# tiantianz/redpanda

Measured on AMD Instinct MI355X. Metric: validated+decoded batch GB/s per GPU and whole node; % of HBM peak, higher is better.
Workload: dtype u8

## Files before the change

redpanda_amd/csrc/rp_device.h:

```cpp
#pragma once

#include "rp_internal.h"

namespace rp {

#define DEV __device__ __forceinline__

DEV uint32_t lane() { return __lane_id(); }

DEV uint32_t wave_xor(uint32_t v) {
#pragma unroll
    for (int o = 32; o > 0; o >>= 1) v ^= __shfl_xor(v, o, 64);
    return v;
}
DEV uint32_t wave_or(uint32_t v) {
#pragma unroll
    for (int o = 32; o > 0; o >>= 1) v |= __shfl_xor(v, o, 64);
    return v;
}
DEV uint32_t rl(uint32_t v, int l) { return (uint32_t)__builtin_amdgcn_readlane((int)v, l); }
DEV uint32_t uni32(uint32_t v) { return (uint32_t)__builtin_amdgcn_readfirstlane((int)v); }
DEV uint64_t uni64(uint64_t v) {
    return (uint64_t)uni32((uint32_t)v) | ((uint64_t)uni32((uint32_t)(v >> 32)) << 32);
}
// ... 138 lines not shown
DEV uint32_t lbe32(const uint32_t (&w)[16], int k) { return __builtin_bswap32(l32(w, k)); }
DEV uint64_t lbe64(const uint32_t (&w)[16], int k) { return ((uint64_t)lbe32(w, k) << 32) | lbe32(w, k + 4); }
DEV uint32_t lbe16(const uint32_t (&w)[16], int k) { return (lb(w, k) << 8) | lb(w, k + 1); }

constexpr int wire_src(int l) {
    return (l >= 8 && l < 16) ? 15 - l
         : (l >= 17 && l < 21) ? 37 - l
         : (l >= 21 && l < 61) ? 21 + ((l < 23 ? 0 : l < 27 ? 2 : l < 35 ? 6 : l < 43 ? 14 : l < 51 ? 22 : l < 53 ? 30
                                        : l < 57 ? 32 : 36) +
                                       ((l < 23 ? 2 : l < 27 ? 4 : l < 35 ? 8 : l < 43 ? 8 : l < 51 ? 8 : l < 53 ? 2
                                        : 4) - 1 - (l - (l < 23 ? 21 : l < 27 ? 23 : l < 35 ? 27 : l < 43 ? 35
                                                         : l < 51 ? 43 : l < 53 ? 51 : l < 57 ? 53 : 57))))
         : 0;
}

DEV LHdr lane_header(uint32_t layout, const uint8_t* __restrict__ seg, uint64_t len, uint64_t p,
                     const uint32_t* __restrict__ th, uint32_t c57) {
    LHdr h;
    h.eof = 0;
    h.hcrc = h.computed = 0;
    h.size = 0;
    h.need = 0;
#pragma unroll
    for (int i = 0; i < 16; i++) h.w[i] = 0;
    const uint64_t rem = len - p;
    if (rem == 0) { h.status = RPGPU_ERRC_END_OF_STREAM; h.eof = 1; return h; }
    if (rem < RPGPU_HEADER_SIZE) { h.status = RPGPU_ERRC_INPUT_STREAM_NOT_ENOUGH_BYTES; h.eof = 1; return h; }
    lane_header_bytes(seg + p, h.w);
    uint32_t raw = 0;
    if (layout == RPGPU_LAYOUT_WIRE) {
        const uint32_t bl = lbe32(h.w, 8);
        if ((int64_t)(int32_t)bl + 12 < (int64_t)RPGPU_HEADER_SIZE) {
            h.status = RPGPU_ERRC_INPUT_STREAM_NOT_ENOUGH_BYTES;
            return h;
        }
        h.size = (int32_t)(bl + 12u);
        h.need = (uint32_t)((uint32_t)h.size - RPGPU_HEADER_SIZE);
#pragma unroll
        for (int k = 4; k < 61; k++) {
            const uint32_t d = (k < 8) ? (((uint32_t)h.size >> (8 * (k - 4))) & 0xFFu) : (k == 16) ? 1u : lb(h.w, wire_src(k));
            raw ^= th[(60 - k) * 256 + d];
        }
        h.computed = ~(c57 ^ raw);
        h.status = -1;
        return h;
    }
#pragma unroll
    for (int k = 4; k < 61; k++) raw ^= th[(60 - k) * 256 + lb(h.w, k)];
    h.computed = ~(c57 ^ raw);
    h.hcrc = h.w[0];
    h.size = (int32_t)h.w[1];
    h.need = (uint32_t)((uint32_t)h.size - RPGPU_HEADER_SIZE);
    if (h.hcrc == 0) { h.status = RPGPU_ERRC_FALLOCATED_FILE_READ_ZERO_BYTES_FOR_HEADER; return h; }
    if (h.hcrc != h.computed) { h.status = RPGPU_ERRC_HEADER_ONLY_CRC_MISSMATCH; return h; }
    h.status = -1;
    return h;
}

DEV uint32_t lane_prefix_raw(uint32_t layout, const uint32_t (&w)[16], const uint32_t* __restrict__ th) {
    uint32_t x = 0;
    if (layout == RPGPU_LAYOUT_WIRE) {
#pragma unroll
        for (int k = 21; k < 61; k++) x ^= th[(39 - (k - 21)) * 256 + lb(w, k)];
    } else {
#pragma unroll
        for (int k = 21; k < 61; k++) x ^= th[(39 - (wire_src(k) - 21)) * 256 + lb(w, k)];
    }
    return x;
}

// ... 134 lines not shown
```

redpanda_amd/csrc/rp_internal.h:

```cpp
#pragma once

#include <hip/hip_runtime.h>
#include <stdint.h>

#include "rpgpu.h"

namespace rp {

constexpr uint64_t kNone = ~0ull;
constexpr uint32_t kCrcPoly = 0x82F63B78u;

constexpr uint32_t kShiftLevels = 6;
constexpr uint32_t kBraidSkip = 1020;

constexpr uint32_t kVWaves = 16;
constexpr uint32_t kWinBytes = 16384;
constexpr uint32_t kLdsBraidOff = 0;
constexpr uint32_t kLdsSlice4Off = 131072;
constexpr uint32_t kLdsShiftOff = kLdsSlice4Off + 4096;
constexpr uint32_t kLdsValidateBytes = kLdsShiftOff + kShiftLevels * 4096;
static_assert(kLdsValidateBytes <= 160u * 1024u, "validate LDS image exceeds 160 KiB");

struct Tables {
    uint32_t slice[4][256];
// ... 119 lines not shown
constexpr size_t kCounterBytes = 256;

struct DeviceJob {
    const uint8_t* data;
    uint64_t data_len;
    const uint64_t* seg_off;
    const uint64_t* chunk_base;
    uint32_t n_segments;
    uint32_t flags;
    uint32_t layout;
    uint32_t chunk_bytes;
    uint32_t total_chunks;
    ChunkRec* chunks;
    uint64_t* chunk_count;
    uint64_t* chunk_entry;
    SegTerm* seg_term;
    rpgpu_batch_result* batches;
    uint64_t batch_capacity;
    uint64_t* slots;
    uint64_t* dcap;
    rpgpu_record_index* records;
    uint64_t record_capacity;
    uint8_t* decoded;
    uint64_t decoded_capacity;
    rpgpu_segment_summary* summaries;
    rpgpu_job_totals* totals;
    uint64_t* bitmap;
    const Tables* tables;
    uint32_t* counters;
    uint32_t* decode_list;
// ... 51 lines not shown
    uint64_t cap;
    uint32_t n;
    uint32_t ord;
    int32_t record_count;
    int32_t status;
};
hipError_t launch_host_desc(const DeviceJob& j, HostItem* items, uint32_t n, hipStream_t s);
hipError_t launch_host_gather(const DeviceJob& j, const HostItem* items, uint32_t n, uint8_t* stage, hipStream_t s);
hipError_t launch_host_patch(const DeviceJob& j, const HostItem* items, uint32_t n, hipStream_t s);
hipError_t launch_host_scatter(const DeviceJob& j, const HostItem* items, uint32_t n, const uint8_t* stage,
                               hipStream_t s);

hipError_t launch_chunk_base(const DeviceJob& j, hipStream_t s);
hipError_t launch_discover(const DeviceJob& j, hipStream_t s);
hipError_t launch_resolve(const DeviceJob& j, hipStream_t s);
hipError_t launch_emit(const DeviceJob& j, hipStream_t s);
hipError_t launch_validate(const DeviceJob& j, hipStream_t s, uint32_t grid, bool compose = true);
hipError_t launch_crc_compose(const DeviceJob& j, hipStream_t s, uint32_t grid);
bool dchain_wanted(const DeviceJob& j);
hipError_t launch_dchain(const DeviceJob& j, hipStream_t s, uint32_t grid);
hipError_t launch_validate_decoded(const DeviceJob& j, hipStream_t s, uint32_t grid);
hipError_t launch_walk(const DeviceJob& j, hipStream_t s, uint32_t grid);
hipError_t launch_decode(const DeviceJob& j, hipStream_t s, uint32_t grid);
hipError_t launch_decode_blocks(const DeviceJob& j, hipStream_t s, uint32_t grid);
hipError_t launch_lz_walk(const DeviceJob& j, hipStream_t s, uint32_t grid);
hipError_t launch_lz_exec(const DeviceJob& j, hipStream_t s);
hipError_t launch_raw_copy(const DeviceJob& j, hipStream_t s, uint32_t cus);
hipError_t launch_lzf_walk(const DeviceJob& j, hipStream_t s, uint32_t cus);
hipError_t launch_decode_finish(const DeviceJob& j, hipStream_t s, uint32_t grid, bool defer = false);
hipError_t launch_content_xxh(const DeviceJob& j, hipStream_t s, uint32_t grid);
hipError_t launch_content_apply(const DeviceJob& j, hipStream_t s, uint32_t grid);
// ... 79 lines not shown
```

redpanda_amd/csrc/rp_kernels.hip:

```cpp
#include "rp_device.h"

namespace rp {


#ifdef RPGPU_CHECKED
#include <cstdio>
#define RP_CHECK(flag, cond, fmt, ...)                                               \
    do {                                                                            \
        if (!(cond)) {                                                              \
            if (__lane_id() == 0) printf("RPGPU_CHECK %d " fmt "\n", __LINE__, __VA_ARGS__); \
            flag = true;                                                            \
        }                                                                           \
    } while (0)
#endif

DEV uint32_t find_segment(const uint64_t* __restrict__ chunk_base, uint32_t nseg, uint64_t g) {
    uint32_t lo = 0, hi = nseg;
    while (hi - lo > 1) {
        uint32_t mid = (lo + hi) >> 1;
        if (chunk_base[mid] <= g) lo = mid; else hi = mid;
    }
    return lo;
}

struct WalkOut {
    uint64_t exit;
    uint64_t tpos;
    uint32_t count;
    int32_t term;
};

DEV WalkOut wave_walk(uint32_t layout, const uint8_t* __restrict__ seg, uint64_t len, uint64_t p, uint64_t ce,
                      const Tables* __restrict__ T) {
    WalkOut w;
    w.count = 0;
    w.term = -1;
    w.tpos = 0;
    while (p < ce) {
        Hdr h = wave_header_of(layout, seg, len, p, T);
        if (h.status >= 0) { w.term = h.status | (h.eof << 8); w.tpos = p; break; }
        if (len - p - RPGPU_HEADER_SIZE < h.need) {
            w.count++;
            w.term = RPGPU_ERRC_INPUT_STREAM_NOT_ENOUGH_BYTES | (1 << 8);
            w.tpos = p;
            break;
        }
        w.count++;
        p += RPGPU_HEADER_SIZE + h.need;
    }
    w.exit = p;
    return w;
}

typedef uint32_t u32x4 __attribute__((ext_vector_type(4)));
struct ScanWin {
// ... 151 lines not shown
        exhausted = entry == kNone && se < ce;
    }
    if (lane() == 0) {
        ChunkRec r;
        r.entry = kNone;
        r.exit = kNone;
        r.count = 0;
        r.term = -1;
        r.tpos = 0;
        j.chunks[g] = r;
        j.chunk_entry[g] = entry != kNone ? entry : exhausted ? kExhausted : kNone;
    }
}

DEV WalkOut lane_walk(uint32_t layout, const uint8_t* __restrict__ seg, uint64_t len, uint64_t p, uint64_t ce,
                      const uint32_t* __restrict__ th, uint32_t c57) {
    WalkOut w;
    w.count = 0;
    w.term = -1;
    w.tpos = 0;
    while (p < ce) {
        const LHdr h = lane_header(layout, seg, len, p, th, c57);
        if (h.status >= 0) { w.term = h.status | (h.eof << 8); w.tpos = p; break; }
        if (len - p - RPGPU_HEADER_SIZE < h.need) {
            w.count++;
            w.term = RPGPU_ERRC_INPUT_STREAM_NOT_ENOUGH_BYTES | (1 << 8);
            w.tpos = p;
            break;
        }
        w.count++;
        p += RPGPU_HEADER_SIZE + h.need;
    }
    w.exit = p;
    return w;
}

__global__ __launch_bounds__(256) void k_chain(DeviceJob j) {
    extern __shared__ uint32_t th[];
// ... 5 lines not shown
    const uint32_t s = find_segment(j.chunk_base, j.n_segments, g);
    const uint64_t w = g - j.chunk_base[s];
    const uint64_t W = j.chunk_base[s + 1] - j.chunk_base[s];
    const uint64_t off = j.seg_off[s], len = j.seg_off[s + 1] - off;
    uint64_t p = entry;
    for (uint32_t k = 0;; k++) {
        const uint64_t cs = (w + k) * j.chunk_bytes;
        const uint64_t ce = (cs + j.chunk_bytes < len) ? cs + j.chunk_bytes : len;
        ChunkRec r;
        r.entry = kNone;
        r.exit = kNone;
        r.count = 0;
        r.term = -1;
        r.tpos = 0;
        if (p < ce) {
            const WalkOut o = lane_walk(j.layout, j.data + off, len, p, ce, th, j.tables->c57);
            r.entry = p;
            r.exit = o.exit;
            r.count = o.count;
            r.term = o.term;
            r.tpos = o.tpos;
            p = o.exit;
        }
        j.chunks[g + k] = r;
        if (r.term >= 0 || k + 1 >= kMaxCarry || w + k + 1 >= W || j.chunk_entry[g + k + 1] != kExhausted) break;
    }
}

__global__ __launch_bounds__(256) void k_resolve(DeviceJob j) {
    const uint32_t s = blockIdx.x;
    const uint32_t tid = threadIdx.x;
// ... 75 lines not shown
            continue;
        }
        const uint64_t wf = w0 + first;
        if (tid == first) s_pred = pred;
        __syncthreads();
        const uint64_t P = s_pred;
        if (tid < 64) {
            const uint64_t cs2 = wf * CS;
            const uint64_t ce2 = (cs2 + CS < len) ? cs2 + CS : len;
            WalkOut o;
            uint64_t entry = kNone;
            if (P >= ce2) {
                o.exit = P; o.count = 0; o.term = -1; o.tpos = 0;
            } else {
                entry = P;
                o = wave_walk(j.layout, seg, len, P, ce2, j.tables);
            }
            if (tid == 0) {
                ChunkRec nr;
                nr.entry = entry; nr.exit = o.exit; nr.count = o.count; nr.term = o.term; nr.tpos = o.tpos;
                j.chunks[c0 + wf] = nr;
                j.chunk_count[c0 + wf] = o.count;
                j.chunk_entry[c0 + wf] = entry;
                atomicAdd(&j.counters[0], 1u);
                if (o.term >= 0) {
                    s_st.pos = o.tpos; s_st.errc = o.term & 0xFF; s_st.eof = (o.term >> 8) & 1;
                    s_ended = 1;
                }
                s_T = o.exit;
            }
        }
        __syncthreads();
        w0 = wf + 1;
    }
    for (uint64_t w = w0 + tid; w < W; w += 256) {
        if (s_ended) {
            j.chunk_count[c0 + w] = 0;
            j.chunk_entry[c0 + w] = kNone;
        }
    }
    if (tid == 0) {
        if (!s_ended) { s_st.pos = s_T; s_st.errc = RPGPU_ERRC_END_OF_STREAM; s_st.eof = 1; }
        j.seg_term[s] = s_st;
    }
}

__global__ __launch_bounds__(256) void k_emit(DeviceJob j) {
    extern __shared__ uint32_t th[];
    init_lds_hdr(th, j.tables);
    const uint64_t g = (uint64_t)blockIdx.x * blockDim.x + threadIdx.x;
    if (g >= j.total_chunks) return;
    const uint64_t base_ord = j.chunk_count[g];
    const uint64_t cnt = j.chunk_count[g + 1] - base_ord;
    if (cnt == 0) return;
    const uint32_t s = find_segment(j.chunk_base, j.n_segments, g);
    const uint64_t off = j.seg_off[s], len = j.seg_off[s + 1] - off;
    const uint8_t* seg = j.data + off;
    const uint32_t c57 = j.tables->c57;
    const bool wire = j.layout == RPGPU_LAYOUT_WIRE;
    uint64_t p = j.chunk_entry[g];
    for (uint64_t i = 0; i < cnt; i++) {
#ifdef RPGPU_CHECKED
        if (!(p < len)) {
            printf("RPGPU_CHECK emit g=%llu i=%llu cnt=%llu p=%llu len=%llu\n", (unsigned long long)g,
                   (unsigned long long)i, (unsigned long long)cnt, (unsigned long long)p, (unsigned long long)len);
            break;
        }
#endif
        const LHdr h = lane_header(j.layout, seg, len, p, th, c57);
        const uint64_t ord = base_ord + i;
        const bool complete = (len - p - RPGPU_HEADER_SIZE) >= h.need;
        const uint32_t praw = lane_prefix_raw(j.layout, h.w, th);
        const uint32_t attrs = wire ? lbe16(h.w, 21) : l16(h.w, 21);
        const int32_t rc = (int32_t)(wire ? lbe32(h.w, 57) : l32(h.w, 57));
        const uint32_t codec = attrs & 7;
        uint64_t slots = 0, cap = 0;
        const bool decodable = (codec == RPGPU_CODEC_LZ4 || codec == RPGPU_CODEC_SNAPPY) && (j.flags & RPGPU_JOB_DECODE);
        if (complete) {
            if (codec == 0) {
                if ((j.flags & RPGPU_JOB_PARSE) && rc > 0 && (uint64_t)rc <= h.need) slots = (uint64_t)rc;
            } else if (decodable) {
                cap = decode_capacity_dev((int)codec, seg + p + RPGPU_HEADER_SIZE, h.need);
                if ((j.flags & RPGPU_JOB_PARSE) && rc > 0 && (uint64_t)rc <= cap) slots = (uint64_t)rc;
            }
        }
        if (ord < j.batch_capacity) {
            rpgpu_batch_result r;
            r.file_pos = p;
            uint32_t f = RPGPU_F_HEADER_OK;
            if (wire) {
                r.base_offset = (int64_t)lbe64(h.w, 0);
                r.first_timestamp = (int64_t)lbe64(h.w, 27);
                r.max_timestamp = (int64_t)lbe64(h.w, 35);
                r.producer_id = (int64_t)lbe64(h.w, 43);
                r.last_offset_delta = (int32_t)lbe32(h.w, 23);
                r.base_sequence = (int32_t)lbe32(h.w, 53);
                r.header_crc = 0;
                r.crc = lbe32(h.w, 17);
                r.producer_epoch = (int16_t)lbe16(h.w, 51);
                r.type = 1;
                if (lb(h.w, 16) == 2) f |= RPGPU_F_WIRE_V2;
            } else {
                r.base_offset = (int64_t)l64(h.w, 8);
                r.first_timestamp = (int64_t)l64(h.w, 27);
                r.max_timestamp = (int64_t)l64(h.w, 35);
                r.producer_id = (int64_t)l64(h.w, 43);
                r.last_offset_delta = (int32_t)l32(h.w, 23);
                r.base_sequence = (int32_t)l32(h.w, 53);
                r.header_crc = h.hcrc;
                r.crc = l32(h.w, 17);
                r.producer_epoch = (int16_t)l16(h.w, 51);
                r.type = (int8_t)lb(h.w, 16);
            }
            r.size_bytes = h.size;
            r.record_count = rc;
            r.crc_computed = 0;
            r.header_crc_computed = h.computed;
            if (complete) f |= RPGPU_F_COMPLETE;
            if (codec) f |= RPGPU_F_COMPRESSED;
            if (codec >= 5) f |= RPGPU_F_CODEC_INVALID;
            const bool host_codec = (j.flags & RPGPU_JOB_DECODE) && (j.flags & RPGPU_JOB_HOST_CODECS);
            if (complete && codec == RPGPU_CODEC_ZSTD && !(j.flags & RPGPU_JOB_DECODE)) f |= RPGPU_F_CODEC_UNSUPPORTED;
            r.flags = f;
            r.segment = s;
            r.index_base = off + p + RPGPU_HEADER_SIZE;
            r.decoded_off = 0;
            r.records_parsed = 0;
            r.decoded_len = (complete && codec == 0) ? (uint32_t)h.need : 0;
            r.decoded_crc = 0;
            r.decoded_header_crc = 0;
            r.attrs = (int16_t)attrs;
            r.parse_err = 0;
            r.reserved0 = 0;
            r.reserved1 = praw;
            j.batches[ord] = r;
            j.slots[ord] = slots;
            j.dcap[ord] = cap;
            if (complete && decodable) j.decode_list[atomicAdd(&j.counters[2], 1u)] = (uint32_t)ord;
            if (complete && (j.flags & RPGPU_JOB_DECODE) &&
                (codec == RPGPU_CODEC_GZIP || (codec == RPGPU_CODEC_ZSTD && !host_codec)))
                j.inf_list[atomicAdd(&j.counters[16], 1u)] = (uint32_t)ord;
            if (complete && codec == RPGPU_CODEC_ZSTD && host_codec)
                j.host_list[atomicAdd(&j.counters[19], 1u)] = (uint32_t)ord;
        }
        if (!complete) break;
        p += RPGPU_HEADER_SIZE + h.need;
    }
}

constexpr uint32_t kScanTile = 4096;

__global__ __launch_bounds__(256) void k_scan_tiles(uint64_t* data, const uint64_t* d_n, uint64_t n_host, uint64_t* tile_sums) {
    const uint64_t n = d_n ? (*d_n < n_host ? *d_n : n_host) : n_host;
    const uint64_t t0 = (uint64_t)blockIdx.x * kScanTile;
    if (t0 >= n) return;
    __shared__ uint64_t s[256];
    uint64_t v[16];
    uint64_t sum = 0;
    const uint64_t b = t0 + threadIdx.x * 16;
#pragma unroll
    for (int i = 0; i < 16; i++) {
// ... 5 lines not shown
    for (int o = 1; o < 256; o <<= 1) {
        uint64_t x = (threadIdx.x >= (uint32_t)o) ? s[threadIdx.x - o] : 0;
        __syncthreads();
        s[threadIdx.x] += x;
        __syncthreads();
    }
    uint64_t run = s[threadIdx.x] - sum;
#pragma unroll
    for (int i = 0; i < 16; i++) {
        if (b + i < n) data[b + i] = run;
        run += v[i];
    }
    if (threadIdx.x == 255) tile_sums[blockIdx.x] = s[255];
}

__global__ __launch_bounds__(1024) void k_scan_sums(uint64_t* tile_sums, const uint64_t* d_n, uint64_t n_host, uint64_t* total_out) {
    const uint64_t n = d_n ? (*d_n < n_host ? *d_n : n_host) : n_host;
    const uint64_t nt = (n + kScanTile - 1) / kScanTile;
    __shared__ uint64_t s[1024];
    __shared__ uint64_t carry;
    if (threadIdx.x == 0) carry = 0;
    __syncthreads();
    for (uint64_t t0 = 0; t0 < nt; t0 += 1024) {
        const uint64_t t = t0 + threadIdx.x;
        uint64_t v = t < nt ? tile_sums[t] : 0;
        s[threadIdx.x] = v;
        __syncthreads();
        for (int o = 1; o < 1024; o <<= 1) {
            uint64_t x = (threadIdx.x >= (uint32_t)o) ? s[threadIdx.x - o] : 0;
            __syncthreads();
            s[threadIdx.x] += x;
            __syncthreads();
        }
        if (t < nt) tile_sums[t] = carry + s[threadIdx.x] - v;
        __syncthreads();
        if (threadIdx.x == 1023) carry += s[1023];
        __syncthreads();
    }
    if (threadIdx.x == 0) total_out[0] = carry;
}

__global__ __launch_bounds__(256) void k_scan_add(uint64_t* data, const uint64_t* d_n, uint64_t n_host, const uint64_t* tile_sums) {
    const uint64_t n = d_n ? (*d_n < n_host ? *d_n : n_host) : n_host;
    const uint64_t t0 = (uint64_t)blockIdx.x * kScanTile;
    if (t0 >= n) return;
    const uint64_t add = tile_sums[blockIdx.x];
    for (uint64_t i = t0 + threadIdx.x; i < t0 + kScanTile && i < n; i += 256) data[i] += add;
}

__global__ __launch_bounds__(256) void k_finalize_segments(DeviceJob j) {
    const uint32_t s = blockIdx.x;
    const uint32_t tid = threadIdx.x;
    const uint64_t first = j.chunk_count[j.chunk_base[s]];
    const uint64_t last = j.chunk_count[j.chunk_base[s + 1]];
    const uint64_t cnt = last - first;
    const bool fits = last <= j.batch_capacity;
    const uint64_t fb = j.seg_first_bad[s];
    const uint64_t bad = (fits && fb < cnt) ? fb : cnt;
    const uint64_t upto = bad < cnt ? bad + (j.layout == RPGPU_LAYOUT_WIRE ? 0 : 1) : cnt;
    const uint64_t seg_len = j.seg_off[s + 1] - j.seg_off[s];
    __shared__ unsigned long long s_bytes, s_phys;
    if (tid == 0) { s_bytes = 0; s_phys = 0; }
    __syncthreads();
    if (fits) {
        if (seg_len < (1ull << 32)) {
            if (tid == 0) {
                if (upto > 0) {
// ... 52 lines not shown
        !(f & RPGPU_F_CODEC_OK))
        return false;
    if ((f & RPGPU_F_PARSED) && !(f & RPGPU_F_PARSE_OK)) return false;
    return true;
}

__global__ __launch_bounds__(256) void k_finalize_bitmap(DeviceJob j) {
    const uint64_t nb_total = j.chunk_count[j.total_chunks];
    const uint64_t nb = nb_total < j.batch_capacity ? nb_total : j.batch_capacity;
    const uint64_t b = (uint64_t)blockIdx.x * 256 + threadIdx.x;
    if ((b & ~63ull) >= nb) return;
    const uint64_t word = __ballot(b < nb && batch_valid(j.batches[b].flags, j.flags, j.layout));
    if ((threadIdx.x & 63) == 0) j.bitmap[b >> 6] = word;
}

__global__ void k_finalize_totals(DeviceJob j) {
    if (threadIdx.x != 0 || blockIdx.x != 0) return;
    const uint64_t nb_total = j.chunk_count[j.total_chunks];
    const uint64_t nb = nb_total < j.batch_capacity ? nb_total : j.batch_capacity;
    rpgpu_job_totals t;
    t.n_batches = nb_total;
    t.n_records = j.slots[nb];
    const uint64_t dtot = (j.flags & RPGPU_JOB_DECODE) ? j.dcap[nb] : 0;
    t.decoded_bytes = dtot;
    t.batch_capacity_needed = nb_total;
    t.record_capacity_needed = j.slots[nb];
    t.decoded_capacity_needed = dtot;
    uint32_t ov = j.counters[1];
    if (nb_total > j.batch_capacity) ov |= 1;
    if (j.slots[nb] > j.record_capacity) ov |= 2;
    if (dtot > j.decoded_capacity) ov |= 4;
    t.overflow = ov;
// ... 66 lines not shown
    return hipGetLastError();
}
hipError_t launch_host_patch(const DeviceJob& j, const HostItem* items, uint32_t n, hipStream_t s) {
    if (n) hipLaunchKernelGGL(k_host_patch, dim3((n + 255) / 256), dim3(256), 0, s, j, items, n);
    return hipGetLastError();
}
hipError_t launch_host_scatter(const DeviceJob& j, const HostItem* items, uint32_t n, const uint8_t* stage,
                               hipStream_t s) {
    if (n) hipLaunchKernelGGL(k_host_scatter, dim3((n + 3) / 4), dim3(256), 0, s, j, items, n, stage);
    return hipGetLastError();
}

__global__ __launch_bounds__(1024) void k_chunk_base(DeviceJob j) {
    __shared__ uint64_t sh[1024];
    __shared__ uint64_t carry;
    if (threadIdx.x == 0) carry = 0;
    __syncthreads();
    for (uint32_t b0 = 0; b0 < j.n_segments; b0 += 1024) {
        const uint32_t i = b0 + threadIdx.x;
        uint64_t v = 0;
        if (i < j.n_segments) {
            const uint64_t len = j.seg_off[i + 1] - j.seg_off[i];
            v = (len + j.chunk_bytes - 1) / j.chunk_bytes;
            if (v == 0) v = 1;
        }
        sh[threadIdx.x] = v;
        __syncthreads();
        for (int o = 1; o < 1024; o <<= 1) {
            uint64_t x = threadIdx.x >= (uint32_t)o ? sh[threadIdx.x - o] : 0;
            __syncthreads();
// ... 12 lines not shown
    hipLaunchKernelGGL(k_chunk_base, dim3(1), dim3(1024), 0, s, j);
    return hipGetLastError();
}

hipError_t launch_discover(const DeviceJob& j, hipStream_t s) {
    hipLaunchKernelGGL(k_discover, dim3((j.total_chunks + 3) / 4), dim3(256), 0, s, j);
    hipError_t e = hipGetLastError();
    if (e != hipSuccess) return e;
    hipLaunchKernelGGL(k_chain, dim3((j.total_chunks + 255) / 256), dim3(256), kLdsHdrBytes, s, j);
    return hipGetLastError();
}
hipError_t launch_resolve(const DeviceJob& j, hipStream_t s) {
    hipLaunchKernelGGL(k_resolve, dim3(j.n_segments), dim3(256), 0, s, j);
    return hipGetLastError();
}
hipError_t launch_emit(const DeviceJob& j, hipStream_t s) {
    hipLaunchKernelGGL(k_emit, dim3((j.total_chunks + 255) / 256), dim3(256), kLdsHdrBytes, s, j);
    return hipGetLastError();
}
hipError_t launch_finalize(const DeviceJob& j, hipStream_t s) {
    hipLaunchKernelGGL(k_finalize_segments, dim3(j.n_segments), dim3(256), 0, s, j);
    const uint64_t words = (j.batch_capacity + 63) / 64;
    if (j.bitmap) {
        const uint32_t grid = (uint32_t)((words * 64 + 255) / 256);
        hipLaunchKernelGGL(k_finalize_bitmap, dim3(grid ? grid : 1), dim3(256), 0, s, j);
    }
    hipLaunchKernelGGL(k_finalize_totals, dim3(1), dim3(64), 0, s, j);
    return hipGetLastError();
}

size_t scan_temp_bytes(uint64_t n) { return ((n + kScanTile - 1) / kScanTile + 1) * sizeof(uint64_t); }

hipError_t scan_exclusive_dev(uint64_t* data, const uint64_t* d_n, uint64_t n_cap, uint64_t* temp, hipStream_t s) {
    const uint32_t tiles = (uint32_t)((n_cap + kScanTile - 1) / kScanTile);
    const uint32_t g = tiles ? tiles : 1;
    hipLaunchKernelGGL(k_scan_tiles, dim3(g), dim3(256), 0, s, data, d_n, n_cap, temp);
    hipLaunchKernelGGL(k_scan_sums, dim3(1), dim3(1024), 0, s, temp, d_n, n_cap, temp + g);
    hipLaunchKernelGGL(k_scan_add, dim3(g), dim3(256), 0, s, data, d_n, n_cap, temp);
    return hipGetLastError();
}

__global__ void k_copy_total(uint64_t* data, const uint64_t* d_n, uint64_t n_host, const uint64_t* total) {
    const uint64_t n = d_n ? (*d_n < n_host ? *d_n : n_host) : n_host;
    data[n] = *total;
}

hipError_t scan_exclusive_u64(uint64_t* data, uint64_t n, void* temp, size_t temp_bytes, hipStream_t s) {
    (void)temp_bytes;
    uint64_t* t = (uint64_t*)temp;
    const uint32_t tiles = (uint32_t)((n + kScanTile - 1) / kScanTile);
    scan_exclusive_dev(data, nullptr, n, t, s);
    hipLaunchKernelGGL(k_copy_total, dim3(1), dim3(1), 0, s, data, (const uint64_t*)nullptr, n, t + (tiles ? tiles : 1));
    return hipGetLastError();
}

hipError_t scan_exclusive_u64_devn(uint64_t* data, const uint64_t* d_n, uint64_t n_cap, void* temp, hipStream_t s) {
    uint64_t* t = (uint64_t*)temp;
    const uint32_t tiles = (uint32_t)((n_cap + kScanTile - 1) / kScanTile);
    scan_exclusive_dev(data, d_n, n_cap, t, s);
    hipLaunchKernelGGL(k_copy_total, dim3(1), dim3(1), 0, s, data, d_n, n_cap, t + (tiles ? tiles : 1));
    return hipGetLastError();
}

}
```

redpanda_amd/csrc/rp_runtime.hip:

```cpp
#include <hip/hip_runtime.h>
#include <nmmintrin.h>

#include <algorithm>
#include <array>
#include <atomic>
#include <cstdio>
#include <cstdlib>
#include <cstring>
#include <mutex>
#include <random>
#include <string>
#include <thread>
#include <vector>

#include "rp_device.h"
#include "rp_hostcodec.h"

namespace rp {

static uint32_t raw_step_zero(uint32_t c, const uint32_t* t0) { return t0[c & 0xFF] ^ (c >> 8); }

static void build_tables(Tables* T) {
    uint32_t t0[256];
    for (uint32_t i = 0; i < 256; i++) {
// ... 575 lines not shown

int check_job(rpgpu_ctx* c, const rpgpu_job* job) {
    if (!c || !job || !job->d_data || !job->d_seg_offsets || !job->h_seg_offsets || job->n_segments == 0 ||
        !job->d_batches || !job->d_summaries || !job->d_totals)
        return fail(c, RPGPU_E_INVALID, "rpgpu_submit: missing argument");
    if (((uintptr_t)job->d_data & 15) != 0) return fail(c, RPGPU_E_INVALID, "rpgpu_submit: d_data must be 16-byte aligned");
    if (job->layout != RPGPU_LAYOUT_DISK && job->layout != RPGPU_LAYOUT_WIRE)
        return fail(c, RPGPU_E_INVALID, "rpgpu_submit: unknown layout");
    if ((job->flags & RPGPU_JOB_PARSE) && !job->d_records && job->record_capacity)
        return fail(c, RPGPU_E_INVALID, "rpgpu_submit: PARSE needs d_records");
    return RPGPU_OK;
}

struct Layout {
    uint64_t tc;
    uint64_t zcap, gcap, bl_cap, split_min, split_cap;
    size_t cbase, chunks, ccount, centry, segterm, slots, dcap, counters, dlist, slist, llist, fbad;
    size_t ilist, istate, ioff, itot, hlist, zitems, gzsmem, gzsit;
    size_t blocks, plans, pstate, longl, wlong, rawl, lanel, lzfl, lzft, split, spart, scan;
    size_t need;
};

Layout job_layout(const rpgpu_job* job, uint32_t cu_count) {
    Layout L;
    const uint32_t nseg = job->n_segments;
    const uint32_t cs = job->chunk_bytes ? job->chunk_bytes : (256u << 10);
    const uint64_t bcap = job->batch_capacity, data_len = job->h_seg_offsets[nseg];
    uint64_t tc = 0;
    for (uint32_t i = 0; i < nseg; i++) {
        const uint64_t len = job->h_seg_offsets[i + 1] - job->h_seg_offsets[i];
        uint64_t nc = (len + cs - 1) / cs;
        tc += nc ? nc : 1;
    }
    L.tc = tc;
    size_t off = 0;
    auto take = [&](size_t bytes) { size_t o = off; off = align_up(off + bytes, 256); return o; };
    L.cbase = take((nseg + 1) * 8);
    L.chunks = take(tc * sizeof(ChunkRec));
    L.ccount = take((tc + 1) * 8);
    L.centry = take(tc * 8);
    L.segterm = take(nseg * sizeof(SegTerm));
    L.slots = take((bcap + 1) * 8);
    L.dcap = take((bcap + 1) * 8);
    L.counters = take(kCounterBytes);
    L.dlist = take((bcap + 1) * 4);
    L.slist = take((bcap + 1) * 4);
    L.llist = take((bcap + 1) * 4);
    L.fbad = take((size_t)nseg * 4);
    const bool decode_job = (job->flags & RPGPU_JOB_DECODE) != 0;
    L.ilist = take(decode_job ? (bcap + 1) * 4 : 0);
    L.istate = take(decode_job ? (bcap + 1) * 4 : 0);
    L.ioff = take(decode_job ? (bcap + 1) * 8 : 0);
    L.itot = take(decode_job ? (bcap + 1) * 8 : 0);
    const bool host_job = decode_job && (job->flags & RPGPU_JOB_HOST_CODECS);
    L.hlist = take(host_job ? (bcap + 1) * 4 : 0);
// ... 38 lines not shown
    if (int rc = grow(c, c->ws, L.need, s, "workspace")) return rc;
    uint8_t* ws = c->ws.as<uint8_t>();

    j.data = job->d_data;
    j.data_len = data_len;
    j.seg_off = job->d_seg_offsets;
    j.chunk_base = (const uint64_t*)(ws + L.cbase);
    j.n_segments = nseg;
    j.flags = job->flags;
    j.layout = job->layout;
    j.chunk_bytes = job->chunk_bytes ? job->chunk_bytes : (256u << 10);
    j.total_chunks = (uint32_t)L.tc;
    j.chunks = (ChunkRec*)(ws + L.chunks);
    j.chunk_count = (uint64_t*)(ws + L.ccount);
    j.chunk_entry = (uint64_t*)(ws + L.centry);
    j.seg_term = (SegTerm*)(ws + L.segterm);
    j.batches = job->d_batches;
    j.batch_capacity = job->batch_capacity;
    j.slots = (uint64_t*)(ws + L.slots);
    j.dcap = (uint64_t*)(ws + L.dcap);
    j.records = job->d_records;
    j.record_capacity = job->d_records ? job->record_capacity : 0;
    j.decoded = job->d_decoded;
    j.decoded_capacity = job->d_decoded ? job->decoded_capacity : 0;
    j.summaries = job->d_summaries;
    j.totals = job->d_totals;
    j.bitmap = job->d_valid_bitmap;
    j.tables = c->d_tables;
    j.counters = (uint32_t*)(ws + L.counters);
    j.decode_list = (uint32_t*)(ws + L.dlist);
// ... 81 lines not shown
        HIPCHK(c, (call));                                                                 \
        if (diag().debug_sync) {                                                           \
            fprintf(stderr, "[rpgpu] stage %s\n", name);                                   \
            fflush(stderr);                                                                \
            hipError_t _e = hipStreamSynchronize(s);                                       \
            if (_e == hipSuccess && c->side.stream) _e = hipStreamSynchronize(c->side.stream);   \
            if (_e == hipSuccess && c->side2.stream) _e = hipStreamSynchronize(c->side2.stream); \
            if (_e != hipSuccess) return fail(c, RPGPU_E_HIP, "stage " name " failed", _e); \
        }                                                                                  \
    } while (0)

hipError_t mark(hipEvent_t* ev, int i, hipStream_t s) { return ev ? hipEventRecord(ev[i], s) : hipSuccess; }

int stage_discover(rpgpu_ctx* c, const DeviceJob& j, hipStream_t s, hipEvent_t* ev, uint64_t* scan_tmp, bool emit) {
    STAGE("chunk_base", launch_chunk_base(j, s));
    HIPCHK(c, hipMemsetAsync(j.counters, 0, kCounterBytes, s));
    HIPCHK(c, hipMemsetAsync(j.seg_first_bad, 0xFF, (size_t)j.n_segments * 4, s));
    STAGE("discover", launch_discover(j, s));
    HIPCHK(c, mark(ev, 1, s));
    STAGE("resolve", launch_resolve(j, s));
    STAGE("scan_chunks", scan_exclusive_u64(j.chunk_count, j.total_chunks, scan_tmp, 0, s));
    if (emit) STAGE("emit", launch_emit(j, s));
    return RPGPU_OK;
}

int stage_members(rpgpu_ctx* c, DeviceJob& j, hipStream_t s, uint64_t* scan_tmp) {
    const uint32_t cus = c->cu_count;
    if (j.flags & RPGPU_JOB_DECODE) {
        const bool split = j.inf_scratch && j.zs_fast;
        STAGE("zstamps", launch_zstamps(s, 0));
        Fork zfork;
        if (split) {
            j.zs_split = 1;
            HIPCHK(c, zfork.open(s, c->side));
            STAGE("zplan", launch_zplan(j, c->side.stream, cus * 4));
            STAGE("zparse", launch_zparse(j, c->side.stream, cus * 4));
            HIPCHK(c, zfork.end());
// ... 834 lines not shown
```

Before: 3600.

## Parallelize batch emit across recorded header positions and fold small launches

During the discover walk, the first K batch-header positions of each chunk are now recorded into a new chunk_pos array. The emit kernel then uses these to spread work across (chunk, index) items in a grid-stride loop with software-prefetched header loads, where previously one thread serially walked each whole chunk. It also removes two memsets by zeroing counters in k_chunk_base, drops the k_copy_total and k_finalize_totals launches by folding them into existing kernels, and stages segment tables in LDS. The cost is extra workspace and stores during the walk, and the K-th item must still walk any remaining batches serially.

```diff
diff --git a/redpanda_amd/csrc/rp_device.h b/redpanda_amd/csrc/rp_device.h
--- a/redpanda_amd/csrc/rp_device.h
+++ b/redpanda_amd/csrc/rp_device.h
@@ -176,6 +176,40 @@
          : 0;
 }
 
+DEV void lane_header_verdict(uint32_t layout, LHdr& h, const uint32_t* __restrict__ th, uint32_t c57) {
+    h.eof = 0;
+    h.hcrc = h.computed = 0;
+    h.size = 0;
+    h.need = 0;
+    uint32_t raw = 0;
+    if (layout == RPGPU_LAYOUT_WIRE) {
+        const uint32_t bl = lbe32(h.w, 8);
+        if ((int64_t)(int32_t)bl + 12 < (int64_t)RPGPU_HEADER_SIZE) {
+            h.status = RPGPU_ERRC_INPUT_STREAM_NOT_ENOUGH_BYTES;
+            return;
+        }
+        h.size = (int32_t)(bl + 12u);
+        h.need = (uint32_t)((uint32_t)h.size - RPGPU_HEADER_SIZE);
+#pragma unroll
+        for (int k = 4; k < 61; k++) {
+            const uint32_t d = (k < 8) ? (((uint32_t)h.size >> (8 * (k - 4))) & 0xFFu) : (k == 16) ? 1u : lb(h.w, wire_src(k));
+            raw ^= th[(60 - k) * 256 + d];
+        }
+        h.computed = ~(c57 ^ raw);
+        h.status = -1;
+        return;
+    }
+#pragma unroll
+    for (int k = 4; k < 61; k++) raw ^= th[(60 - k) * 256 + lb(h.w, k)];
+    h.computed = ~(c57 ^ raw);
+    h.hcrc = h.w[0];
+    h.size = (int32_t)h.w[1];
+    h.need = (uint32_t)((uint32_t)h.size - RPGPU_HEADER_SIZE);
+    if (h.hcrc == 0) { h.status = RPGPU_ERRC_FALLOCATED_FILE_READ_ZERO_BYTES_FOR_HEADER; return; }
+    if (h.hcrc != h.computed) { h.status = RPGPU_ERRC_HEADER_ONLY_CRC_MISSMATCH; return; }
+    h.status = -1;
+}
+
 DEV LHdr lane_header(uint32_t layout, const uint8_t* __restrict__ seg, uint64_t len, uint64_t p,
                      const uint32_t* __restrict__ th, uint32_t c57) {
     LHdr h;
@@ -189,33 +223,7 @@
     if (rem == 0) { h.status = RPGPU_ERRC_END_OF_STREAM; h.eof = 1; return h; }
     if (rem < RPGPU_HEADER_SIZE) { h.status = RPGPU_ERRC_INPUT_STREAM_NOT_ENOUGH_BYTES; h.eof = 1; return h; }
     lane_header_bytes(seg + p, h.w);
-    uint32_t raw = 0;
-    if (layout == RPGPU_LAYOUT_WIRE) {
-        const uint32_t bl = lbe32(h.w, 8);
-        if ((int64_t)(int32_t)bl + 12 < (int64_t)RPGPU_HEADER_SIZE) {
-            h.status = RPGPU_ERRC_INPUT_STREAM_NOT_ENOUGH_BYTES;
-            return h;
-        }
-        h.size = (int32_t)(bl + 12u);
-        h.need = (uint32_t)((uint32_t)h.size - RPGPU_HEADER_SIZE);
-#pragma unroll
-        for (int k = 4; k < 61; k++) {
-            const uint32_t d = (k < 8) ? (((uint32_t)h.size >> (8 * (k - 4))) & 0xFFu) : (k == 16) ? 1u : lb(h.w, wire_src(k));
-            raw ^= th[(60 - k) * 256 + d];
-        }
-        h.computed = ~(c57 ^ raw);
-        h.status = -1;
-        return h;
-    }
-#pragma unroll
-    for (int k = 4; k < 61; k++) raw ^= th[(60 - k) * 256 + lb(h.w, k)];
-    h.computed = ~(c57 ^ raw);
-    h.hcrc = h.w[0];
-    h.size = (int32_t)h.w[1];
-    h.need = (uint32_t)((uint32_t)h.size - RPGPU_HEADER_SIZE);
-    if (h.hcrc == 0) { h.status = RPGPU_ERRC_FALLOCATED_FILE_READ_ZERO_BYTES_FOR_HEADER; return h; }
-    if (h.hcrc != h.computed) { h.status = RPGPU_ERRC_HEADER_ONLY_CRC_MISSMATCH; return h; }
-    h.status = -1;
+    lane_header_verdict(layout, h, th, c57);
     return h;
 }
 
diff --git a/redpanda_amd/csrc/rp_internal.h b/redpanda_amd/csrc/rp_internal.h
--- a/redpanda_amd/csrc/rp_internal.h
+++ b/redpanda_amd/csrc/rp_internal.h
@@ -157,6 +157,8 @@
     ChunkRec* chunks;
     uint64_t* chunk_count;
     uint64_t* chunk_entry;
+    uint32_t* chunk_pos;
+    uint32_t chunk_pos_k;
     SegTerm* seg_term;
     rpgpu_batch_result* batches;
     uint64_t batch_capacity;
@@ -238,7 +240,7 @@
 hipError_t launch_chunk_base(const DeviceJob& j, hipStream_t s);
 hipError_t launch_discover(const DeviceJob& j, hipStream_t s);
 hipError_t launch_resolve(const DeviceJob& j, hipStream_t s);
-hipError_t launch_emit(const DeviceJob& j, hipStream_t s);
+hipError_t launch_emit(const DeviceJob& j, hipStream_t s, uint32_t cus);
 hipError_t launch_validate(const DeviceJob& j, hipStream_t s, uint32_t grid, bool compose = true);
 hipError_t launch_crc_compose(const DeviceJob& j, hipStream_t s, uint32_t grid);
 bool dchain_wanted(const DeviceJob& j);
diff --git a/redpanda_amd/csrc/rp_kernels.hip b/redpanda_amd/csrc/rp_kernels.hip
--- a/redpanda_amd/csrc/rp_kernels.hip
+++ b/redpanda_amd/csrc/rp_kernels.hip
@@ -31,7 +31,7 @@
 };
 
 DEV WalkOut wave_walk(uint32_t layout, const uint8_t* __restrict__ seg, uint64_t len, uint64_t p, uint64_t ce,
-                      const Tables* __restrict__ T) {
+                      const Tables* __restrict__ T, uint32_t* __restrict__ pos, uint64_t ps, uint32_t K, uint64_t cs) {
     WalkOut w;
     w.count = 0;
     w.term = -1;
@@ -39,6 +39,7 @@
     while (p < ce) {
         Hdr h = wave_header_of(layout, seg, len, p, T);
         if (h.status >= 0) { w.term = h.status | (h.eof << 8); w.tpos = p; break; }
+        if (w.count < K && lane() == 0) pos[w.count * ps] = (uint32_t)(p - cs);
         if (len - p - RPGPU_HEADER_SIZE < h.need) {
             w.count++;
             w.term = RPGPU_ERRC_INPUT_STREAM_NOT_ENOUGH_BYTES | (1 << 8);
@@ -220,7 +221,8 @@
 }
 
 DEV WalkOut lane_walk(uint32_t layout, const uint8_t* __restrict__ seg, uint64_t len, uint64_t p, uint64_t ce,
-                      const uint32_t* __restrict__ th, uint32_t c57) {
+                      const uint32_t* __restrict__ th, uint32_t c57, uint32_t* __restrict__ pos, uint64_t ps,
+                      uint32_t K, uint64_t cs) {
     WalkOut w;
     w.count = 0;
     w.term = -1;
@@ -228,6 +230,7 @@
     while (p < ce) {
         const LHdr h = lane_header(layout, seg, len, p, th, c57);
         if (h.status >= 0) { w.term = h.status | (h.eof << 8); w.tpos = p; break; }
+        if (w.count < K) pos[w.count * ps] = (uint32_t)(p - cs);
         if (len - p - RPGPU_HEADER_SIZE < h.need) {
             w.count++;
             w.term = RPGPU_ERRC_INPUT_STREAM_NOT_ENOUGH_BYTES | (1 << 8);
@@ -263,7 +266,8 @@
         r.term = -1;
         r.tpos = 0;
         if (p < ce) {
-            const WalkOut o = lane_walk(j.layout, j.data + off, len, p, ce, th, j.tables->c57);
+            const WalkOut o = lane_walk(j.layout, j.data + off, len, p, ce, th, j.tables->c57,
+                                        j.chunk_pos + (g + k), j.total_chunks, j.chunk_pos_k, cs);
             r.entry = p;
             r.exit = o.exit;
             r.count = o.count;
@@ -369,7 +373,8 @@
                 o.exit = P; o.count = 0; o.term = -1; o.tpos = 0;
             } else {
                 entry = P;
-                o = wave_walk(j.layout, seg, len, P, ce2, j.tables);
+                o = wave_walk(j.layout, seg, len, P, ce2, j.tables, j.chunk_pos + (c0 + wf), j.total_chunks,
+                              j.chunk_pos_k, cs2);
             }
             if (tid == 0) {
                 ChunkRec nr;
@@ -400,106 +405,190 @@
     }
 }
 
+DEV bool emit_batch(const DeviceJob& j, const uint32_t* __restrict__ th, const LHdr& h, uint32_t s, uint64_t off,
+                    uint64_t len, uint64_t p, uint64_t ord) {
+    const uint8_t* seg = j.data + off;
+    const bool wire = j.layout == RPGPU_LAYOUT_WIRE;
+    const bool complete = (len - p - RPGPU_HEADER_SIZE) >= h.need;
+    const uint32_t praw = lane_prefix_raw(j.layout, h.w, th);
+    const uint32_t attrs = wire ? lbe16(h.w, 21) : l16(h.w, 21);
+    const int32_t rc = (int32_t)(wire ? lbe32(h.w, 57) : l32(h.w, 57));
+    const uint32_t codec = attrs & 7;
+    uint64_t slots = 0, cap = 0;
+    const bool decodable = (codec == RPGPU_CODEC_LZ4 || codec == RPGPU_CODEC_SNAPPY) && (j.flags & RPGPU_JOB_DECODE);
+    if (complete) {
+        if (codec == 0) {
+            if ((j.flags & RPGPU_JOB_PARSE) && rc > 0 && (uint64_t)rc <= h.need) slots = (uint64_t)rc;
+        } else if (decodable) {
+            cap = decode_capacity_dev((int)codec, seg + p + RPGPU_HEADER_SIZE, h.need);
+            if ((j.flags & RPGPU_JOB_PARSE) && rc > 0 && (uint64_t)rc <= cap) slots = (uint64_t)rc;
+        }
+    }
+    if (ord < j.batch_capacity) {
+        rpgpu_batch_result r;
+        r.file_pos = p;
+        uint32_t f = RPGPU_F_HEADER_OK;
+        if (wire) {
+            r.base_offset = (int64_t)lbe64(h.w, 0);
+            r.first_timestamp = (int64_t)lbe64(h.w, 27);
+            r.max_timestamp = (int64_t)lbe64(h.w, 35);
+            r.producer_id = (int64_t)lbe64(h.w, 43);
+            r.last_offset_delta = (int32_t)lbe32(h.w, 23);
+            r.base_sequence = (int32_t)lbe32(h.w, 53);
+            r.header_crc = 0;
+            r.crc = lbe32(h.w, 17);
+            r.producer_epoch = (int16_t)lbe16(h.w, 51);
+            r.type = 1;
+            if (lb(h.w, 16) == 2) f |= RPGPU_F_WIRE_V2;
+        } else {
+            r.base_offset = (int64_t)l64(h.w, 8);
+            r.first_timestamp = (int64_t)l64(h.w, 27);
+            r.max_timestamp = (int64_t)l64(h.w, 35);
+            r.producer_id = (int64_t)l64(h.w, 43);
+            r.last_offset_delta = (int32_t)l32(h.w, 23);
+            r.base_sequence = (int32_t)l32(h.w, 53);
+            r.header_crc = h.hcrc;
+            r.crc = l32(h.w, 17);
+            r.producer_epoch = (int16_t)l16(h.w, 51);
+            r.type = (int8_t)lb(h.w, 16);
+        }
+        r.size_bytes = h.size;
+        r.record_count = rc;
+        r.crc_computed = 0;
+        r.header_crc_computed = h.computed;
+        if (complete) f |= RPGPU_F_COMPLETE;
+        if (codec) f |= RPGPU_F_COMPRESSED;
+        if (codec >= 5) f |= RPGPU_F_CODEC_INVALID;
+        const bool host_codec = (j.flags & RPGPU_JOB_DECODE) && (j.flags & RPGPU_JOB_HOST_CODECS);
+        if (complete && codec == RPGPU_CODEC_ZSTD && !(j.flags & RPGPU_JOB_DECODE)) f |= RPGPU_F_CODEC_UNSUPPORTED;
+        r.flags = f;
+        r.segment = s;
+        r.index_base = off + p + RPGPU_HEADER_SIZE;
+        r.decoded_off = 0;
+        r.records_parsed = 0;
+        r.decoded_len = (complete && codec == 0) ? (uint32_t)h.need : 0;
+        r.decoded_crc = 0;
+        r.decoded_header_crc = 0;
+        r.attrs = (int16_t)attrs;
+        r.parse_err = 0;
+        r.reserved0 = 0;
+        r.reserved1 = praw;
+        j.batches[ord] = r;
+        j.slots[ord] = slots;
+        j.dcap[ord] = cap;
+        if (complete && decodable) j.decode_list[atomicAdd(&j.counters[2], 1u)] = (uint32_t)ord;
+        if (complete && (j.flags & RPGPU_JOB_DECODE) &&
+            (codec == RPGPU_CODEC_GZIP || (codec == RPGPU_CODEC_ZSTD && !host_codec)))
+            j.inf_list[atomicAdd(&j.counters[16], 1u)] = (uint32_t)ord;
+        if (complete && codec == RPGPU_CODEC_ZSTD && host_codec)
+            j.host_list[atomicAdd(&j.counters[19], 1u)] = (uint32_t)ord;
+    }
+    return complete;
+}
+
+constexpr uint32_t kEmitSegs = 512;
+constexpr uint32_t kEmitWgsPerCu = 2;
+
+struct EmitRaw {
+    uint64_t c0, c1;
+    uint32_t pos;
+};
+struct EmitItem {
+    uint64_t ord, p, off, len, cnt;
+    uint32_t s, i;
+    bool live;
+};
+
 __global__ __launch_bounds__(256) void k_emit(DeviceJob j) {
     extern __shared__ uint32_t th[];
+    __shared__ uint64_t s_cb[kEmitSegs + 1], s_so[kEmitSegs + 1];
+    const bool staged = j.n_segments <= kEmitSegs;
+    if (staged)
+        for (uint32_t k = threadIdx.x; k <= j.n_segments; k += 256) { s_cb[k] = j.chunk_base[k]; s_so[k] = j.seg_off[k]; }
     init_lds_hdr(th, j.tables);
-    const uint64_t g = (uint64_t)blockIdx.x * blockDim.x + threadIdx.x;
-    if (g >= j.total_chunks) return;
-    const uint64_t base_ord = j.chunk_count[g];
-    const uint64_t cnt = j.chunk_count[g + 1] - base_ord;
-    if (cnt == 0) return;
-    const uint32_t s = find_segment(j.chunk_base, j.n_segments, g);
-    const uint64_t off = j.seg_off[s], len = j.seg_off[s + 1] - off;
-    const uint8_t* seg = j.data + off;
+    const uint64_t* cb = staged ? s_cb : j.chunk_base;
+    const uint64_t* so = staged ? s_so : j.seg_off;
     const uint32_t c57 = j.tables->c57;
-    const bool wire = j.layout == RPGPU_LAYOUT_WIRE;
-    uint64_t p = j.chunk_entry[g];
-    for (uint64_t i = 0; i < cnt; i++) {
+    const uint32_t K = j.chunk_pos_k;
+    const uint64_t n_items = (uint64_t)j.total_chunks * K;
+    const uint64_t stride = (uint64_t)gridDim.x * 256;
+    const uint64_t tc = j.total_chunks;
+
+    auto load_raw = [&](uint64_t it) {
+        EmitRaw r;
+        r.c0 = r.c1 = 0;
+        r.pos = 0;
+        if (it < n_items) {
+            const uint64_t g = it % tc;
+            r.c0 = j.chunk_count[g];
+            r.c1 = j.chunk_count[g + 1];
+            r.pos = j.chunk_pos[it];
+        }
+        return r;
+    };
+    auto resolve = [&](uint64_t it, const EmitRaw& r) {
+        const uint32_t i = (uint32_t)(it / tc);
+        const uint64_t g = it % tc;
+        EmitItem m;
+        m.cnt = r.c1 - r.c0;
+        m.live = i < m.cnt;
+        m.ord = r.c0 + i;
+        m.i = i;
+        m.s = 0;
+        m.p = m.off = m.len = 0;
+        if (m.live) {
+            m.s = find_segment(cb, j.n_segments, g);
+            m.off = so[m.s];
+            m.len = so[m.s + 1] - m.off;
+            m.p = (g - cb[m.s]) * j.chunk_bytes + r.pos;
+        }
+        return m;
+    };
+
+    uint64_t it = (uint64_t)blockIdx.x * 256 + threadIdx.x;
+    EmitItem cur = resolve(it, load_raw(it));
+    LHdr h;
+#pragma unroll
+    for (int k = 0; k < 16; k++) h.w[k] = 0;
+    if (cur.live) lane_header_bytes(j.data + cur.off + cur.p, h.w);
+    EmitRaw rn = load_raw(it + stride);
+    while (it < n_items) {
+        const EmitItem nxt = resolve(it + stride, rn);
+        uint32_t wn[16];
+#pragma unroll
+        for (int k = 0; k < 16; k++) wn[k] = 0;
+        if (nxt.live) lane_header_bytes(j.data + nxt.off + nxt.p, wn);
+        rn = load_raw(it + 2 * stride);
+        if (cur.live) {
 #ifdef RPGPU_CHECKED
-        if (!(p < len)) {
-            printf("RPGPU_CHECK emit g=%llu i=%llu cnt=%llu p=%llu len=%llu\n", (unsigned long long)g,
-                   (unsigned long long)i, (unsigned long long)cnt, (unsigned long long)p, (unsigned long long)len);
-            break;
-        }
+            if (!(cur.p < cur.len))
+                printf("RPGPU_CHECK emit ord=%llu i=%u cnt=%llu p=%llu len=%llu\n", (unsigned long long)cur.ord, cur.i,
+                       (unsigned long long)cur.cnt, (unsigned long long)cur.p, (unsigned long long)cur.len);
 #endif
-        const LHdr h = lane_header(j.layout, seg, len, p, th, c57);
-        const uint64_t ord = base_ord + i;
-        const bool complete = (len - p - RPGPU_HEADER_SIZE) >= h.need;
-        const uint32_t praw = lane_prefix_raw(j.layout, h.w, th);
-        const uint32_t attrs = wire ? lbe16(h.w, 21) : l16(h.w, 21);
-        const int32_t rc = (int32_t)(wire ? lbe32(h.w, 57) : l32(h.w, 57));
-        const uint32_t codec = attrs & 7;
-        uint64_t slots = 0, cap = 0;
-        const bool decodable = (codec == RPGPU_CODEC_LZ4 || codec == RPGPU_CODEC_SNAPPY) && (j.flags & RPGPU_JOB_DECODE);
-        if (complete) {
-            if (codec == 0) {
-                if ((j.flags & RPGPU_JOB_PARSE) && rc > 0 && (uint64_t)rc <= h.need) slots = (uint64_t)rc;
-            } else if (decodable) {
-                cap = decode_capacity_dev((int)codec, seg + p + RPGPU_HEADER_SIZE, h.need);
-                if ((j.flags & RPGPU_JOB_PARSE) && rc > 0 && (uint64_t)rc <= cap) slots = (uint64_t)rc;
+            lane_header_verdict(j.layout, h, th, c57);
+            bool complete = emit_batch(j, th, h, cur.s, cur.off, cur.len, cur.p, cur.ord);
+            if (cur.i == K - 1) {
+                uint64_t p = cur.p, ord = cur.ord;
+                for (uint64_t n = K; n < cur.cnt && complete; n++) {
+                    p += RPGPU_HEADER_SIZE + h.need;
+                    ord++;
+#ifdef RPGPU_CHECKED
+                    if (!(p < cur.len)) {
+                        printf("RPGPU_CHECK emit tail ord=%llu n=%llu cnt=%llu p=%llu len=%llu\n", (unsigned long long)ord,
+                               (unsigned long long)n, (unsigned long long)cur.cnt, (unsigned long long)p,
+                               (unsigned long long)cur.len);
+                        break;
+                    }
+#endif
+                    h = lane_header(j.layout, j.data + cur.off, cur.len, p, th, c57);
+                    complete = emit_batch(j, th, h, cur.s, cur.off, cur.len, p, ord);
+                }
             }
         }
-        if (ord < j.batch_capacity) {
-            rpgpu_batch_result r;
-            r.file_pos = p;
-            uint32_t f = RPGPU_F_HEADER_OK;
-            if (wire) {
-                r.base_offset = (int64_t)lbe64(h.w, 0);
-                r.first_timestamp = (int64_t)lbe64(h.w, 27);
-                r.max_timestamp = (int64_t)lbe64(h.w, 35);
-                r.producer_id = (int64_t)lbe64(h.w, 43);
-                r.last_offset_delta = (int32_t)lbe32(h.w, 23);
-                r.base_sequence = (int32_t)lbe32(h.w, 53);
-                r.header_crc = 0;
-                r.crc = lbe32(h.w, 17);
-                r.producer_epoch = (int16_t)lbe16(h.w, 51);
-                r.type = 1;
-                if (lb(h.w, 16) == 2) f |= RPGPU_F_WIRE_V2;
-            } else {
-                r.base_offset = (int64_t)l64(h.w, 8);
-                r.first_timestamp = (int64_t)l64(h.w, 27);
-                r.max_timestamp = (int64_t)l64(h.w, 35);
-                r.producer_id = (int64_t)l64(h.w, 43);
-                r.last_offset_delta = (int32_t)l32(h.w, 23);
-                r.base_sequence = (int32_t)l32(h.w, 53);
-                r.header_crc = h.hcrc;
-                r.crc = l32(h.w, 17);
-                r.producer_epoch = (int16_t)l16(h.w, 51);
-                r.type = (int8_t)lb(h.w, 16);
-            }
-            r.size_bytes = h.size;
-            r.record_count = rc;
-            r.crc_computed = 0;
-            r.header_crc_computed = h.computed;
-            if (complete) f |= RPGPU_F_COMPLETE;
-            if (codec) f |= RPGPU_F_COMPRESSED;
-            if (codec >= 5) f |= RPGPU_F_CODEC_INVALID;
-            const bool host_codec = (j.flags & RPGPU_JOB_DECODE) && (j.flags & RPGPU_JOB_HOST_CODECS);
-            if (complete && codec == RPGPU_CODEC_ZSTD && !(j.flags & RPGPU_JOB_DECODE)) f |= RPGPU_F_CODEC_UNSUPPORTED;
-            r.flags = f;
-            r.segment = s;
-            r.index_base = off + p + RPGPU_HEADER_SIZE;
-            r.decoded_off = 0;
-            r.records_parsed = 0;
-            r.decoded_len = (complete && codec == 0) ? (uint32_t)h.need : 0;
-            r.decoded_crc = 0;
-            r.decoded_header_crc = 0;
-            r.attrs = (int16_t)attrs;
-            r.parse_err = 0;
-            r.reserved0 = 0;
-            r.reserved1 = praw;
-            j.batches[ord] = r;
-            j.slots[ord] = slots;
-            j.dcap[ord] = cap;
-            if (complete && decodable) j.decode_list[atomicAdd(&j.counters[2], 1u)] = (uint32_t)ord;
-            if (complete && (j.flags & RPGPU_JOB_DECODE) &&
-                (codec == RPGPU_CODEC_GZIP || (codec == RPGPU_CODEC_ZSTD && !host_codec)))
-                j.inf_list[atomicAdd(&j.counters[16], 1u)] = (uint32_t)ord;
-            if (complete && codec == RPGPU_CODEC_ZSTD && host_codec)
-                j.host_list[atomicAdd(&j.counters[19], 1u)] = (uint32_t)ord;
-        }
-        if (!complete) break;
-        p += RPGPU_HEADER_SIZE + h.need;
+        cur = nxt;
+#pragma unroll
+        for (int k = 0; k < 16; k++) h.w[k] = wn[k];
+        it += stride;
     }
 }
 
@@ -535,7 +624,7 @@
     if (threadIdx.x == 255) tile_sums[blockIdx.x] = s[255];
 }
 
-__global__ __launch_bounds__(1024) void k_scan_sums(uint64_t* tile_sums, const uint64_t* d_n, uint64_t n_host, uint64_t* total_out) {
+__global__ __launch_bounds__(1024) void k_scan_sums(uint64_t* tile_sums, const uint64_t* d_n, uint64_t n_host, uint64_t* data) {
     const uint64_t n = d_n ? (*d_n < n_host ? *d_n : n_host) : n_host;
     const uint64_t nt = (n + kScanTile - 1) / kScanTile;
     __shared__ uint64_t s[1024];
@@ -558,7 +647,7 @@
         if (threadIdx.x == 1023) carry += s[1023];
         __syncthreads();
     }
-    if (threadIdx.x == 0) total_out[0] = carry;
+    if (threadIdx.x == 0) data[n] = carry;
 }
 
 __global__ __launch_bounds__(256) void k_scan_add(uint64_t* data, const uint64_t* d_n, uint64_t n_host, const uint64_t* tile_sums) {
@@ -569,9 +658,15 @@
     for (uint64_t i = t0 + threadIdx.x; i < t0 + kScanTile && i < n; i += 256) data[i] += add;
 }
 
+DEV void finalize_totals(const DeviceJob& j);
+
 __global__ __launch_bounds__(256) void k_finalize_segments(DeviceJob j) {
     const uint32_t s = blockIdx.x;
     const uint32_t tid = threadIdx.x;
+    if (s == j.n_segments) {
+        if (tid == 0) finalize_totals(j);
+        return;
+    }
     const uint64_t first = j.chunk_count[j.chunk_base[s]];
     const uint64_t last = j.chunk_count[j.chunk_base[s + 1]];
     const uint64_t cnt = last - first;
@@ -654,8 +749,7 @@
     if ((threadIdx.x & 63) == 0) j.bitmap[b >> 6] = word;
 }
 
-__global__ void k_finalize_totals(DeviceJob j) {
-    if (threadIdx.x != 0 || blockIdx.x != 0) return;
+DEV void finalize_totals(const DeviceJob& j) {
     const uint64_t nb_total = j.chunk_count[j.total_chunks];
     const uint64_t nb = nb_total < j.batch_capacity ? nb_total : j.batch_capacity;
     rpgpu_job_totals t;
@@ -752,6 +846,8 @@
 __global__ __launch_bounds__(1024) void k_chunk_base(DeviceJob j) {
     __shared__ uint64_t sh[1024];
     __shared__ uint64_t carry;
+    if (threadIdx.x < kCounterBytes / 4) j.counters[threadIdx.x] = 0;
+    for (uint32_t i = threadIdx.x; i < j.n_segments; i += 1024) j.seg_first_bad[i] = 0xFFFFFFFFu;
     if (threadIdx.x == 0) carry = 0;
     __syncthreads();
     for (uint32_t b0 = 0; b0 < j.n_segments; b0 += 1024) {
@@ -794,18 +890,19 @@
     hipLaunchKernelGGL(k_resolve, dim3(j.n_segments), dim3(256), 0, s, j);
     return hipGetLastError();
 }
-hipError_t launch_emit(const DeviceJob& j, hipStream_t s) {
-    hipLaunchKernelGGL(k_emit, dim3((j.total_chunks + 255) / 256), dim3(256), kLdsHdrBytes, s, j);
+hipError_t launch_emit(const DeviceJob& j, hipStream_t s, uint32_t cus) {
+    const uint64_t wgs = ((uint64_t)j.total_chunks * j.chunk_pos_k + 255) / 256;
+    const uint64_t grid = wgs < (uint64_t)cus * kEmitWgsPerCu ? wgs : (uint64_t)cus * kEmitWgsPerCu;
+    hipLaunchKernelGGL(k_emit, dim3((uint32_t)(grid ? grid : 1)), dim3(256), kLdsHdrBytes, s, j);
     return hipGetLastError();
 }
 hipError_t launch_finalize(const DeviceJob& j, hipStream_t s) {
-    hipLaunchKernelGGL(k_finalize_segments, dim3(j.n_segments), dim3(256), 0, s, j);
+    hipLaunchKernelGGL(k_finalize_segments, dim3(j.n_segments + 1), dim3(256), 0, s, j);
     const uint64_t words = (j.batch_capacity + 63) / 64;
     if (j.bitmap) {
         const uint32_t grid = (uint32_t)((words * 64 + 255) / 256);
         hipLaunchKernelGGL(k_finalize_bitmap, dim3(grid ? grid : 1), dim3(256), 0, s, j);
     }
-    hipLaunchKernelGGL(k_finalize_totals, dim3(1), dim3(64), 0, s, j);
     return hipGetLastError();
 }
 
@@ -815,31 +912,18 @@
     const uint32_t tiles = (uint32_t)((n_cap + kScanTile - 1) / kScanTile);
     const uint32_t g = tiles ? tiles : 1;
     hipLaunchKernelGGL(k_scan_tiles, dim3(g), dim3(256), 0, s, data, d_n, n_cap, temp);
-    hipLaunchKernelGGL(k_scan_sums, dim3(1), dim3(1024), 0, s, temp, d_n, n_cap, temp + g);
+    hipLaunchKernelGGL(k_scan_sums, dim3(1), dim3(1024), 0, s, temp, d_n, n_cap, data);
     hipLaunchKernelGGL(k_scan_add, dim3(g), dim3(256), 0, s, data, d_n, n_cap, temp);
     return hipGetLastError();
 }
 
-__global__ void k_copy_total(uint64_t* data, const uint64_t* d_n, uint64_t n_host, const uint64_t* total) {
-    const uint64_t n = d_n ? (*d_n < n_host ? *d_n : n_host) : n_host;
-    data[n] = *total;
-}
-
 hipError_t scan_exclusive_u64(uint64_t* data, uint64_t n, void* temp, size_t temp_bytes, hipStream_t s) {
     (void)temp_bytes;
-    uint64_t* t = (uint64_t*)temp;
-    const uint32_t tiles = (uint32_t)((n + kScanTile - 1) / kScanTile);
-    scan_exclusive_dev(data, nullptr, n, t, s);
-    hipLaunchKernelGGL(k_copy_total, dim3(1), dim3(1), 0, s, data, (const uint64_t*)nullptr, n, t + (tiles ? tiles : 1));
-    return hipGetLastError();
+    return scan_exclusive_dev(data, nullptr, n, (uint64_t*)temp, s);
 }
 
 hipError_t scan_exclusive_u64_devn(uint64_t* data, const uint64_t* d_n, uint64_t n_cap, void* temp, hipStream_t s) {
-    uint64_t* t = (uint64_t*)temp;
-    const uint32_t tiles = (uint32_t)((n_cap + kScanTile - 1) / kScanTile);
-    scan_exclusive_dev(data, d_n, n_cap, t, s);
-    hipLaunchKernelGGL(k_copy_total, dim3(1), dim3(1), 0, s, data, d_n, n_cap, t + (tiles ? tiles : 1));
-    return hipGetLastError();
-}
-
-}
+    return scan_exclusive_dev(data, d_n, n_cap, (uint64_t*)temp, s);
+}
+
+}
diff --git a/redpanda_amd/csrc/rp_runtime.hip b/redpanda_amd/csrc/rp_runtime.hip
--- a/redpanda_amd/csrc/rp_runtime.hip
+++ b/redpanda_amd/csrc/rp_runtime.hip
@@ -613,8 +613,9 @@
 
 struct Layout {
     uint64_t tc;
+    uint32_t pos_k;
     uint64_t zcap, gcap, bl_cap, split_min, split_cap;
-    size_t cbase, chunks, ccount, centry, segterm, slots, dcap, counters, dlist, slist, llist, fbad;
+    size_t cbase, chunks, ccount, centry, cpos, segterm, slots, dcap, counters, dlist, slist, llist, fbad;
     size_t ilist, istate, ioff, itot, hlist, zitems, gzsmem, gzsit;
     size_t blocks, plans, pstate, longl, wlong, rawl, lanel, lzfl, lzft, split, spart, scan;
     size_t need;
@@ -638,6 +639,8 @@
     L.chunks = take(tc * sizeof(ChunkRec));
     L.ccount = take((tc + 1) * 8);
     L.centry = take(tc * 8);
+    L.pos_k = std::min<uint32_t>(std::max<uint32_t>(cs / 8192u, 1u), 32u);
+    L.cpos = take(tc * L.pos_k * 4);
     L.segterm = take(nseg * sizeof(SegTerm));
     L.slots = take((bcap + 1) * 8);
     L.dcap = take((bcap + 1) * 8);
@@ -706,6 +709,8 @@
     j.chunks = (ChunkRec*)(ws + L.chunks);
     j.chunk_count = (uint64_t*)(ws + L.ccount);
     j.chunk_entry = (uint64_t*)(ws + L.centry);
+    j.chunk_pos = (uint32_t*)(ws + L.cpos);
+    j.chunk_pos_k = L.pos_k;
     j.seg_term = (SegTerm*)(ws + L.segterm);
     j.batches = job->d_batches;
     j.batch_capacity = job->batch_capacity;
@@ -817,13 +822,11 @@
 
 int stage_discover(rpgpu_ctx* c, const DeviceJob& j, hipStream_t s, hipEvent_t* ev, uint64_t* scan_tmp, bool emit) {
     STAGE("chunk_base", launch_chunk_base(j, s));
-    HIPCHK(c, hipMemsetAsync(j.counters, 0, kCounterBytes, s));
-    HIPCHK(c, hipMemsetAsync(j.seg_first_bad, 0xFF, (size_t)j.n_segments * 4, s));
     STAGE("discover", launch_discover(j, s));
     HIPCHK(c, mark(ev, 1, s));
     STAGE("resolve", launch_resolve(j, s));
     STAGE("scan_chunks", scan_exclusive_u64(j.chunk_count, j.total_chunks, scan_tmp, 0, s));
-    if (emit) STAGE("emit", launch_emit(j, s));
+    if (emit) STAGE("emit", launch_emit(j, s, c->cu_count));
     return RPGPU_OK;
 }
 
```

New measurement: 3436. -4.6%, worse.
